# MDAnalysis/transport-analysis

Measured on AMD Instinct MI355X. Metric: VACF lag-points/sec (n_frames x n_atoms / s), higher is better.
Workload: dtype f64

## Files before the change

### transport_analysis_amd/csrc/wfft.hpp

```cpp
#pragma once
#include <hip/hip_runtime.h>

#include <type_traits>
#include <utility>

#include "fft_engine.hpp"

namespace ta {

#ifndef WF_NW_R0
#define WF_NW_R0 0
#define WF_NW_VAL 0
#endif

template <int LO, int HI, class F>
__device__ __forceinline__ void static_for_range(F&& f) {
    [&]<int... I>(std::integer_sequence<int, I...>) {
        (f(std::integral_constant<int, LO + I>{}), ...);
    }(std::make_integer_sequence<int, (HI > LO ? HI - LO : 0)>{});
}

typedef unsigned int wf_u32x4 __attribute__((ext_vector_type(4)));

#include "wfft_twist.inc"

template <>
struct Dft<3> {
    static __device__ __forceinline__ void run(cd (&v)[3]) {
        constexpr double kS3 = 0.86602540378443864676372317075294;
        const cd t = v[1] + v[2], d = v[1] - v[2];
        const cd m = cd{v[0].x - 0.5 * t.x, v[0].y - 0.5 * t.y};
        const cd e = cd{kS3 * d.y, -kS3 * d.x};
        v[0] = v[0] + t;
        v[1] = m + e;
        v[2] = m - e;
    }
};

template <int N>
struct DftOddTables;
template <>
struct DftOddTables<7> {
    static constexpr double c[3] = {0.62348980185873353053, -0.22252093395631440429, -0.90096886790241912624};
    static constexpr double s[3] = {0.78183148246802980871, 0.97492791218182360702, 0.43388373911755812048};
};
template <>
struct DftOddTables<9> {
    static constexpr double c[4] = {0.76604444311897803520, 0.17364817766693034885, -0.5, -0.93969262078590838405};
    static constexpr double s[4] = {0.64278760968653932632, 0.98480775301220805937, 0.86602540378443864676,
                                    0.34202014332566873304};
};
template <int N>
__device__ __forceinline__ void dft_odd(cd (&v)[N]) {
    constexpr int H = N / 2;
    using Tb = DftOddTables<N>;
    cd sp[H], dm[H];
#pragma unroll
    for (int j = 1; j <= H; ++j) {
        sp[j - 1] = v[j] + v[N - j];
        dm[j - 1] = v[j] - v[N - j];
    }
    const cd x0 = v[0];
    cd sum = x0;
#pragma unroll
    for (int j = 0; j < H; ++j) sum = sum + sp[j];
    v[0] = sum;
#pragma unroll
    for (int k = 1; k <= H; ++k) {
        double rx = x0.x, ry = x0.y, ix = 0.0, iy = 0.0;
#pragma unroll
        for (int j = 1; j <= H; ++j) {
            const int m = (j * k) % N;
            const double cm = m == 0 ? 1.0 : Tb::c[(m <= H ? m : N - m) - 1];
            const double sm = m == 0 ? 0.0 : m <= H ? Tb::s[m - 1] : -Tb::s[N - m - 1];
            rx = fma(cm, sp[j - 1].x, rx);
            ry = fma(cm, sp[j - 1].y, ry);
            ix = fma(sm, dm[j - 1].x, ix);
            iy = fma(sm, dm[j - 1].y, iy);
        }
        v[k] = cd{rx + iy, ry - ix};
        v[N - k] = cd{rx - iy, ry + ix};
    }
}
template <>
struct Dft<7> {
    static __device__ __forceinline__ void run(cd (&v)[7]) { dft_odd<7>(v); }
};
template <>
struct Dft<9> {
    static __device__ __forceinline__ void run(cd (&v)[9]) { dft_odd<9>(v); }
};

template <int N2>
__device__ __forceinline__ void dft_2x(cd (&v)[2 * N2]) {
    constexpr int N = 2 * N2;
    cd s[2][N2];
#pragma unroll
    for (int j2 = 0; j2 < N2; ++j2) {
        const cd a = v[(2 * j2) % N], b = v[(N2 + 2 * j2) % N];
        s[0][j2] = a + b;
        s[1][j2] = a - b;
    }
    Dft<N2>::run(s[0]);
    Dft<N2>::run(s[1]);
#pragma unroll
    for (int q = 0; q < N; ++q) v[q] = s[q % 2][q % N2];
}
template <>
struct Dft<14> {
    static __device__ __forceinline__ void run(cd (&v)[14]) { dft_2x<7>(v); }
};
template <>
struct Dft<18> {
    static __device__ __forceinline__ void run(cd (&v)[18]) { dft_2x<9>(v); }
};

template <>
struct Dft<6> {
    static __device__ __forceinline__ void run(cd (&v)[6]) {
        cd s[2][3];
#pragma unroll
        for (int j2 = 0; j2 < 3; ++j2) {
            const cd a = v[(2 * j2) % 6], b = v[(3 + 2 * j2) % 6];
            s[0][j2] = a + b;
            s[1][j2] = a - b;
        }
        Dft<3>::run(s[0]);
        Dft<3>::run(s[1]);
#pragma unroll
        for (int q = 0; q < 6; ++q) v[q] = s[q % 2][q % 3];
    }
};

template <>
struct Dft<12> {
    static __device__ __forceinline__ void run(cd (&v)[12]) {
        cd s[4][3];
#pragma unroll
        for (int j2 = 0; j2 < 3; ++j2) {
            cd t[4] = {v[(4 * j2) % 12], v[(3 + 4 * j2) % 12], v[(6 + 4 * j2) % 12], v[(9 + 4 * j2) % 12]};
            Dft<4>::run(t);
#pragma unroll
            for (int k1 = 0; k1 < 4; ++k1) s[k1][j2] = t[k1];
        }
#pragma unroll
        for (int k1 = 0; k1 < 4; ++k1) Dft<3>::run(s[k1]);
#pragma unroll
        for (int q = 0; q < 12; ++q) v[q] = s[q % 4][q % 3];
    }
};

template <>
struct Dft<10> {
    static __device__ __forceinline__ void run(cd (&v)[10]) {
        cd s[2][5];
#pragma unroll
        for (int j2 = 0; j2 < 5; ++j2) {
            const cd a = v[(2 * j2) % 10], b = v[(5 + 2 * j2) % 10];
            s[0][j2] = a + b;
            s[1][j2] = a - b;
        }
        Dft<5>::run(s[0]);
        Dft<5>::run(s[1]);
#pragma unroll
        for (int q = 0; q < 10; ++q) v[q] = s[q % 2][q % 5];
    }
};

template <>
struct Dft<20> {
    static __device__ __forceinline__ void run(cd (&v)[20]) {
        cd s[4][5];
#pragma unroll
        for (int j2 = 0; j2 < 5; ++j2) {
            cd t[4] = {v[(4 * j2) % 20], v[(5 + 4 * j2) % 20], v[(10 + 4 * j2) % 20], v[(15 + 4 * j2) % 20]};
            Dft<4>::run(t);
#pragma unroll
            for (int k1 = 0; k1 < 4; ++k1) s[k1][j2] = t[k1];
        }
#pragma unroll
        for (int k1 = 0; k1 < 4; ++k1) Dft<5>::run(s[k1]);
#pragma unroll
        for (int q = 0; q < 20; ++q) v[q] = s[q % 4][q % 5];
    }
};

constexpr int kWfStageRows = 14 + 8;
inline size_t wf_table_elems(int R0, int R) { return 2 * (size_t)R * R0 * 512 + kWfStageRows * 64; }
inline cd wf_tan_form(long num, long den) {
    const long double pi = 3.141592653589793238462643383279502884L;
    num %= den;
    if (4 * num == den) return cd{-0x1p200, 0x1p-200};
    if (4 * num == 3 * den) return cd{0x1p200, 0x1p-200};
    if (num == 0) return cd{0.0, 1.0};
    if (2 * num == den) return cd{0.0, -1.0};
    const long double h = 2.0L * pi * (long double)num / (long double)den;
    const long double c = cosl(h), sn = -sinl(h);
    return cd{(double)(sn / c), (double)c};
}
inline void wf_fill_table(int R0, int R, cd* a) {
    const long L = 2L * R * R0 * 512;
    const long double pi = 3.141592653589793238462643383279502884L;
    for (long n = 0; n < L; ++n) {
        if (n == 0) a[n] = cd{1.0, 0.0};
        else if (2 * n == L) a[n] = cd{-1.0, 0.0};
        else if (4 * n == L) a[n] = cd{0.0, -1.0};
        else if (4 * n == 3 * L) a[n] = cd{0.0, 1.0};
        else {
            const long double h = 2.0L * pi * (long double)n / (long double)L;
            a[n] = cd{(double)cosl(h), (double)-sinl(h)};
        }
    }
    for (int r = 1; r < 8; ++r)
        for (int l = 0; l < 64; ++l) {
            a[L + (r - 1) * 64 + l] = a[(L / 512) * l * r];
            a[L + (6 + r) * 64 + l] = a[(L / 64) * (l & 7) * r];
        }
    cd* t = a + L + 14 * 64;
    for (int l = 0; l < 64; ++l) {
        const long gb = 8 * (l >> 3), gc = 8 * (l & 7) + (l >> 3);
        const long g[2] = {gb, gc};
        for (int st = 0; st < 2; ++st) {
            t[(4 * st + 0) * 64 + l] = wf_tan_form(4 * g[st], 512);
            t[(4 * st + 1) * 64 + l] = wf_tan_form(2 * g[st], 512);
            t[(4 * st + 2) * 64 + l] = wf_tan_form(g[st], 512);
            t[(4 * st + 3) * 64 + l] = wf_tan_form(g[st] + 64, 512);
        }
    }
}

template <int R0_>
struct WPlan {
    static constexpr int R0 = R0_;
    static constexpr int N1 = 512;
    static constexpr int NW = R0 == WF_NW_R0 ? WF_NW_VAL : R0 <= 4 ? 2 : R0 <= 7 ? 4 : 8;
    static constexpr int NT = 64 * NW;
    static constexpr int K1 = (N1 + NT - 1) / NT;
#ifndef WF_SPREAD_ALL
    static constexpr bool kSpreadRows = R0 >= 9 && R0 <= 16;
#else
    static constexpr bool kSpreadRows = WF_SPREAD_ALL && (R0 < 18 || R0 == WF_NW_R0);
#endif
#ifndef WF_REG_EXCHANGE
    static constexpr bool kRegExchange = R0 >= 16;
#else
    static constexpr bool kRegExchange = WF_REG_EXCHANGE;
#endif
#ifndef WF_REG_EXCHANGE_SINGLE
    static constexpr bool kRegExchangeSingle = R0 == 2 || R0 == 7 || R0 == 9 || R0 == 10 || R0 == 12 || R0 == 14;
#else
    static constexpr bool kRegExchangeSingle = (WF_REG_EXCHANGE_SINGLE >> (R0 - 1)) & 1;
#endif
#ifndef WF_MINW_R0
    static __host__ __device__ constexpr int min_waves(bool , bool lng) { return R0 == 2 ? 4 : 1; }
#else
    static __host__ __device__ constexpr int min_waves(bool, bool) { return R0 == WF_MINW_R0 ? WF_MINW_VAL : 1; }
#endif
    static constexpr bool kTwResident = true;
    static constexpr int M = R0 * N1;
    static constexpr int NS1 = (R0 + NW - 1) / NW;
    static constexpr int NLO = R0 / NW, REM = R0 % NW;
    static __host__ __device__ constexpr int sub_count(int wave) { return NLO + (wave < REM ? 1 : 0); }
    static __host__ __device__ constexpr int sub_base(int wave) { return wave * NLO + (wave < REM ? wave : REM); }
    static constexpr size_t kLds = (size_t)M * sizeof(cd);

    struct RealSel {
        unsigned qmask[2];
        unsigned q1mask[2];
    };
    static __host__ __device__ constexpr int owner(int q) {
        for (int w = 0; w < NW; ++w)
            if (q >= sub_base(w) && q < sub_base(w) + sub_count(w)) return w;
        return 0;
    }
    static __host__ __device__ constexpr RealSel real_selection() {
        RealSel r{{0u, 0u}, {0u, 0u}};
        for (int t = 0; t < 2; ++t) {
            int load[8] = {0, 0, 0, 0, 0, 0, 0, 0}, simd[4] = {0, 0, 0, 0};
            auto take = [&](int q, bool self) {
                r.qmask[t] |= 1u << q;
                if (self) r.q1mask[t] |= 1u << q;
                ++load[owner(q)];
                ++simd[owner(q) % 4];
            };
            const int span = t == 0 ? R0 : R0 - 1;
            for (int q = 0; q < R0; ++q)
                if ((span - q + R0) % R0 == q) take(q, true);
            for (int q = 0; q < R0; ++q) {
                const int m = (span - q + R0) % R0;
                if (m <= q) continue;
                const int wa = owner(q), wb = owner(m);
                const int ca = 16 * load[wa] + simd[wa % 4], cb = 16 * load[wb] + simd[wb % 4];
                take(cb < ca ? m : q, false);
            }
        }
        return r;
    }
    static constexpr RealSel kRealSel = real_selection();
};

__device__ __forceinline__ cd wf_load(__amdgpu_buffer_rsrc_t r, unsigned lane_off, unsigned uni_off) {
    const wf_u32x4 v = __builtin_amdgcn_raw_buffer_load_b128(r, lane_off, uni_off, 0);
    return __builtin_bit_cast(cd, v);
}

struct WfSubPost {
    int lane, hi, lo;
    __device__ __forceinline__ explicit WfSubPost(int lane_) : lane(lane_) {
        asm volatile("" : "+v"(lane));
        hi = lane >> 3;
        lo = lane & 7;
    }
    __device__ __forceinline__ void read_a(const cd* __restrict__ reg, cd (&v)[8]) const {
#pragma unroll
        for (int n2 = 0; n2 < 8; ++n2) v[n2] = reg[64 * n2 + lane];
    }
    __device__ __forceinline__ void stage_a(cd* __restrict__ reg, cd (&v)[8], const cd (&twa)[7]) const {
        Dft<8>::run(v);
#pragma unroll
        for (int a = 1; a < 8; ++a) v[a] = cmul(v[a], twa[a - 1]);
        __builtin_amdgcn_wave_barrier();
#pragma unroll
        for (int a = 0; a < 8; ++a) reg[a * 64 + (lane ^ (8 * (a & 1)))] = v[a];
        __builtin_amdgcn_wave_barrier();
        const int base = hi * 64 + (lo ^ (8 * (hi & 1)));
#pragma unroll
        for (int n1 = 0; n1 < 8; ++n1) v[n1] = reg[base ^ (8 * n1)];
        __builtin_amdgcn_wave_barrier();
    }
    __device__ __forceinline__ void stage_b(cd* __restrict__ reg, cd (&v)[8], const cd (&twb)[7]) const {
        Dft<8>::run(v);
#pragma unroll
        for (int b = 1; b < 8; ++b) v[b] = cmul(v[b], twb[b - 1]);
        __builtin_amdgcn_wave_barrier();
        const int x = lo ^ hi;
#pragma unroll
        for (int b = 0; b < 8; ++b) reg[(hi * 8 + b) * 8 + (x ^ b)] = v[b];
        __builtin_amdgcn_wave_barrier();
#pragma unroll
        for (int n0 = 0; n0 < 8; ++n0) v[n0] = reg[lane * 8 + (n0 ^ x)];
        __builtin_amdgcn_wave_barrier();
    }
    __device__ __forceinline__ void stage_c(cd (&v)[8], double (&acc)[8]) const {
        Dft<8>::run(v);
#pragma unroll
        for (int c = 0; c < 8; ++c) acc[c] = fma(v[c].y, v[c].y, fma(v[c].x, v[c].x, acc[c]));
        __builtin_amdgcn_wave_barrier();
    }
};

template <int ROT>
__device__ __forceinline__ void wf_bf(cd& A, cd& B, const cd t) {
    const double qx = fma(-t.x, B.y, B.x), qy = fma(t.x, B.x, B.y);
    const cd a = A;
    if constexpr (ROT == 0) {
        A = cd{fma(t.y, qx, a.x), fma(t.y, qy, a.y)};
        B = cd{fma(-t.y, qx, a.x), fma(-t.y, qy, a.y)};
    } else {
        A = cd{fma(t.y, qy, a.x), fma(-t.y, qx, a.y)};
        B = cd{fma(-t.y, qy, a.x), fma(t.y, qx, a.y)};
    }
}
__device__ __forceinline__ void wf_dft8_tw(cd (&v)[8], const cd (&t)[4]) {
    wf_bf<0>(v[0], v[4], t[0]);
    wf_bf<0>(v[1], v[5], t[0]);
    wf_bf<0>(v[2], v[6], t[0]);
    wf_bf<0>(v[3], v[7], t[0]);
    wf_bf<0>(v[0], v[2], t[1]);
    wf_bf<0>(v[1], v[3], t[1]);
    wf_bf<1>(v[4], v[6], t[1]);
    wf_bf<1>(v[5], v[7], t[1]);
    wf_bf<0>(v[0], v[1], t[2]);
    wf_bf<1>(v[2], v[3], t[2]);
    wf_bf<0>(v[4], v[5], t[3]);
    wf_bf<1>(v[6], v[7], t[3]);
    const cd y4 = v[1], y6 = v[3], y1 = v[4], y3 = v[6];
    v[1] = y1, v[3] = y3, v[4] = y4, v[6] = y6;
}

struct WfTw {
    cd b[4], c[4];
};
typedef unsigned wf_u32pair __attribute__((ext_vector_type(2)));
__device__ __forceinline__ void wf_transpose_hi(cd (&v)[8]) {
    unsigned w[8][4];
#pragma unroll
    for (int a = 0; a < 8; ++a) {
        const wf_u32x4 t = __builtin_bit_cast(wf_u32x4, v[a]);
        w[a][0] = t.x, w[a][1] = t.y, w[a][2] = t.z, w[a][3] = t.w;
    }
#pragma unroll
    for (int a = 0; a < 8; ++a)
        if (!(a & 4))
#pragma unroll
            for (int d = 0; d < 4; ++d) {
                const wf_u32pair r = __builtin_amdgcn_permlane32_swap(w[a][d], w[a | 4][d], false, false);
                w[a][d] = r.x, w[a | 4][d] = r.y;
            }
#pragma unroll
    for (int a = 0; a < 8; ++a)
        if (!(a & 2))
#pragma unroll
            for (int d = 0; d < 4; ++d) {
                const wf_u32pair r = __builtin_amdgcn_permlane16_swap(w[a][d], w[a | 2][d], false, false);
                w[a][d] = r.x, w[a | 2][d] = r.y;
            }
#pragma unroll
    for (int a = 0; a < 8; ++a)
        if (!(a & 1))
#pragma unroll
            for (int d = 0; d < 4; ++d) {
                const unsigned lo = w[a][d], hi = w[a | 1][d];
                w[a][d] = __builtin_amdgcn_update_dpp(lo, hi, 0x128, 0xF, 0xC, false);
                w[a | 1][d] = __builtin_amdgcn_update_dpp(hi, lo, 0x128, 0xF, 0x3, false);
            }
#pragma unroll
    for (int a = 0; a < 8; ++a) {
        wf_u32x4 t;
        t.x = w[a][0], t.y = w[a][1], t.z = w[a][2], t.w = w[a][3];
        v[a] = __builtin_bit_cast(cd, t);
    }
}

struct WfAddr {
    unsigned we, wo, re, ro, x16, b2w, b2r;
    __device__ __forceinline__ void init(int lane, unsigned q_bytes) {
        const int hi = lane >> 3, lo = lane & 7;
        we = q_bytes + 16u * (unsigned)lane;
        wo = q_bytes + 16u * (unsigned)(lane ^ 8);
        const unsigned rb = q_bytes + 16u * (unsigned)(hi * 64 + lo);
        re = rb + 128u * (unsigned)(hi & 1);
        ro = rb - 128u * (unsigned)(hi & 1);
        x16 = 16u * (unsigned)(hi ^ lo);
        b2w = q_bytes + 1024u * (unsigned)hi;
        b2r = b2w + 128u * (unsigned)lo;
    }
    __device__ __forceinline__ unsigned w2(int k) const { return (x16 ^ (16u * (unsigned)k)) + b2w; }
    __device__ __forceinline__ unsigned r2(int k) const { return (x16 ^ (16u * (unsigned)k)) + b2r; }
};
struct WfSub {
    const WfAddr& ad;
    unsigned char* smem;
    __device__ __forceinline__ WfSub(const WfAddr& ad_, unsigned char* smem_) : ad(ad_), smem(smem_) {}
    __device__ __forceinline__ cd& at(unsigned base, unsigned off) const {
        return *reinterpret_cast<cd*>(__builtin_assume_aligned(smem + (base + off), 16));
    }
    template <unsigned SO>
    __device__ __forceinline__ void read_a(cd (&v)[8]) const {
#pragma unroll
        for (int n2 = 0; n2 < 8; ++n2) v[n2] = at(ad.we, SO + 1024u * n2);
    }
    template <unsigned SO>
    __device__ __forceinline__ void stage_a_w(cd (&v)[8]) const {
        Dft<8>::run(v);
        __builtin_amdgcn_wave_barrier();
#pragma unroll
        for (int a = 0; a < 8; ++a) at(a & 1 ? ad.wo : ad.we, SO + 1024u * a) = v[a];
        __builtin_amdgcn_wave_barrier();
    }
    template <unsigned SO>
    __device__ __forceinline__ void stage_a_r(cd (&v)[8]) const {
        __builtin_amdgcn_wave_barrier();
#pragma unroll
        for (int n1 = 0; n1 < 8; ++n1) v[n1] = at(n1 & 1 ? ad.ro : ad.re, SO + 128u * n1);
        __builtin_amdgcn_wave_barrier();
    }
    template <unsigned SO, bool XV = false>
    __device__ __forceinline__ void stage_a(cd (&v)[8]) const {
        if constexpr (XV) {
            Dft<8>::run(v);
            wf_transpose_hi(v);
        } else {
            stage_a_w<SO>(v);
            stage_a_r<SO>(v);
        }
    }
    template <unsigned SO>
    __device__ __forceinline__ void stage_b_w(cd (&v)[8], const WfTw& tw) const {
        wf_dft8_tw(v, tw.b);
        __builtin_amdgcn_wave_barrier();
#pragma unroll
        for (int b = 0; b < 8; ++b) at(ad.w2(b), SO + 128u * b) = v[b];
        __builtin_amdgcn_wave_barrier();
    }
    template <unsigned SO>
    __device__ __forceinline__ void stage_b_r(cd (&v)[8]) const {
        __builtin_amdgcn_wave_barrier();
#pragma unroll
        for (int n0 = 0; n0 < 8; ++n0) v[n0] = at(ad.r2(n0), SO);
        __builtin_amdgcn_wave_barrier();
    }
    template <unsigned SO>
    __device__ __forceinline__ void stage_b(cd (&v)[8], const WfTw& tw) const {
        stage_b_w<SO>(v, tw);
        stage_b_r<SO>(v);
    }
    __device__ __forceinline__ void stage_c(cd (&v)[8], const WfTw& tw, double (&acc)[8]) const {
        wf_dft8_tw(v, tw.c);
#pragma unroll
        for (int c = 0; c < 8; ++c) acc[c] = fma(v[c].y, v[c].y, fma(v[c].x, v[c].x, acc[c]));
    }
    __device__ __forceinline__ void stage_c_w(cd (&v)[8], const WfTw& tw, double (&acc)[8], double wgt) const {
        wf_dft8_tw(v, tw.c);
#pragma unroll
        for (int c = 0; c < 8; ++c) acc[c] = fma(wgt, fma(v[c].y, v[c].y, v[c].x * v[c].x), acc[c]);
    }
};

constexpr unsigned kWfSubBytes = 512 * sizeof(cd);

struct WfNoHook {
    template <class T>
    __device__ __forceinline__ void operator()(T) const {}
};
template <int I>
using wf_part = std::integral_constant<int, I>;

template <int S0, bool XV = false, class Hook = WfNoHook>
__device__ __forceinline__ void wf_sub512(const WfSub& w, const WfTw& tw, double (&acc)[8], Hook&& hook = Hook{}) {
    cd v[8];
    w.read_a<S0 * kWfSubBytes>(v);
    hook(wf_part<0>{});
    w.template stage_a<S0 * kWfSubBytes, XV>(v);
    hook(wf_part<1>{});
    w.stage_b<S0 * kWfSubBytes>(v, tw);
    hook(wf_part<2>{});
    w.stage_c(v, tw, acc);
    hook(wf_part<3>{});
}

template <int S0, bool XV = false>
__device__ __forceinline__ void wf_sub512_w(const WfSub& w, const WfTw& tw, double (&acc)[8], double wgt) {
    cd v[8];
    w.read_a<S0 * kWfSubBytes>(v);
    w.template stage_a<S0 * kWfSubBytes, XV>(v);
    w.stage_b<S0 * kWfSubBytes>(v, tw);
    w.stage_c_w(v, tw, acc, wgt);
}

template <int S0, bool XV = false, class Hook = WfNoHook>
__device__ __forceinline__ void wf_sub512_x2(const WfSub& w, const WfTw& tw, double (&acc0)[8],
                                             double (&acc1)[8], Hook&& hook = Hook{}) {
    constexpr unsigned A = S0 * kWfSubBytes, B = A + kWfSubBytes;
    cd v0[8], v1[8];
    w.read_a<A>(v0);
    w.read_a<B>(v1);
    __builtin_amdgcn_wave_barrier();
    hook(wf_part<0>{});
    w.template stage_a<A>(v0);
    w.template stage_a<B, XV>(v1);
    hook(wf_part<1>{});
    w.stage_b<A>(v0, tw);
    w.stage_b<B>(v1, tw);
    hook(wf_part<2>{});
    w.stage_c(v0, tw, acc0);
    w.stage_c(v1, tw, acc1);
    hook(wf_part<3>{});
}

template <bool XV = false, class Hook = WfNoHook>
__device__ __forceinline__ void wf_sub512_x3(const WfSub& w, const WfTw& tw, double (&acc0)[8],
                                             double (&acc1)[8], double (&acc2)[8], Hook&& hook = Hook{}) {
    constexpr unsigned A = 0, B = kWfSubBytes, C = 2 * kWfSubBytes;
    cd v0[8], v1[8], v2[8];
    w.read_a<A>(v0);
    w.read_a<B>(v1);
    w.read_a<C>(v2);
    __builtin_amdgcn_wave_barrier();
    hook(wf_part<0>{});
    w.template stage_a<A>(v0);
    w.template stage_a<B>(v1);
    w.template stage_a<C, XV>(v2);
    hook(wf_part<1>{});
    w.stage_b<A>(v0, tw);
    w.stage_b<B>(v1, tw);
    w.stage_b<C>(v2, tw);
    hook(wf_part<2>{});
    w.stage_c(v0, tw, acc0);
    w.stage_c(v1, tw, acc1);
    w.stage_c(v2, tw, acc2);
    hook(wf_part<3>{});
}

__device__ __forceinline__ void wf_unit_of(long atom, int k, int D, long* pair, int* kind) {
    const long c0 = atom * D;
    if (D == 2) {
        *pair = atom, *kind = 2;
    } else if (D == 1) {
        *pair = c0 >> 1, *kind = (int)(c0 & 1);
    } else if ((c0 & 1) == 0) {
        *pair = (c0 >> 1) + k, *kind = k == 0 ? 2 : 0;
    } else {
        *pair = (c0 >> 1) + k, *kind = k == 0 ? 1 : 2;
    }
}

typedef unsigned int wf_u32x2 __attribute__((__vector_size__(2 * sizeof(unsigned int))));

__device__ __forceinline__ cd wf_cfma(cd acc, cd a, cd b) {
    return {acc.x + (a.x * b.x - a.y * b.y), acc.y + (a.x * b.y + a.y * b.x)};
}

template <bool S, class A, class B>
__device__ __forceinline__ auto& wf_pick(A& a, B& b) {
    if constexpr (S) return a;
    else return b;
}

template <class P, bool BYP = false, bool LONG = false, bool STAMP = false, bool SRC32 = false>
__global__ void __launch_bounds__(P::NT, P::min_waves(BYP, LONG))
    k_wsplit_accum(const double* __restrict__ pm, long pitch, int T, long n_units,
                   const cd* __restrict__ tw2, double* __restrict__ accg, int D, int R_arg,
                   unsigned long long* __restrict__ stamps) {
    extern __shared__ __attribute__((aligned(16))) unsigned char smem_raw[];
    cd* lds = reinterpret_cast<cd*>(smem_raw);
    constexpr int R0 = P::R0, N1 = P::N1, NW = P::NW, NS1 = P::NS1, M = P::M;
    static_assert(!(SRC32 && LONG), "float32 slabs: plans without an outer radix only");
    const int R = LONG ? R_arg : 1, npass = 2 * R, L = npass * M;
    const int tid = threadIdx.x, wave = tid >> 6;
    int lane = tid & 63;
    const int bi = blockIdx.x >> 3;
    const int pass = bi % npass;
    const long tuple = (blockIdx.x & 7) + 8 * (bi / npass), n_tuples = gridDim.x / npass;
    const int upa = BYP ? (D == 3 ? 2 : 1) : 1;
    const int grp = BYP && (D & 1) ? 2 : 1;

    double acc[NS1][8];
#pragma unroll
    for (int s = 0; s < NS1; ++s)
#pragma unroll
        for (int c = 0; c < 8; ++c) acc[s][c] = 0.0;
    unsigned long long st_acc[4] = {0, 0, 0, 0}, st_prev = 0, st_t0 = 0, st_r0 = 0, st_tail = 0, st_s2end = 0;
    if constexpr (STAMP) {
        st_prev = st_t0 = __builtin_amdgcn_s_memtime();
        st_r0 = __builtin_amdgcn_s_memrealtime();
    }
#define WF_STAMP(i)                                                   \
    if constexpr (STAMP) {                                            \
        const unsigned long long now_ = __builtin_amdgcn_s_memtime(); \
        st_acc[i] += now_ - st_prev;                                  \
        st_prev = now_;                                               \
    }
    const __amdgpu_buffer_rsrc_t twr =
        __builtin_amdgcn_make_buffer_rsrc(const_cast<cd*>(tw2), 0, (L + kWfStageRows * 64) * 16, 0x00020000);
    auto unit_rsrc = [&](long item, int k, int* kind) {
        long pair = item;
        const bool live = item < n_units;
        *kind = 2;
        if constexpr (BYP) wf_unit_of(live ? item : 0, k, D, &pair, kind);
        if constexpr (SRC32)
            return __builtin_amdgcn_make_buffer_rsrc(
                const_cast<float*>(reinterpret_cast<const float*>(pm) + (live ? pair : 0) * pitch * 2), 0,
                live ? T * 8 : 0, 0x00020000);
        else
            return __builtin_amdgcn_make_buffer_rsrc(const_cast<double*>(pm + (live ? pair : 0) * pitch * 2), 0,
                                                     live ? T * 16 : 0, 0x00020000);
    };
    using RowT = std::conditional_t<SRC32, wf_u32x2, cd>;
    auto load_row = [&](__amdgpu_buffer_rsrc_t rs, int kd, int u, unsigned row_off) -> RowT {
        if constexpr (SRC32) {
            return __builtin_amdgcn_raw_buffer_load_b64(rs, (unsigned)u * 8u, row_off * 8u, 0);
        } else {
            if (!BYP || kd == 2) return wf_load(rs, (unsigned)u * 16u, row_off * 16u);
            return cd{__builtin_bit_cast(double, __builtin_amdgcn_raw_buffer_load_b64(
                                                     rs, (unsigned)u * 16u + (unsigned)kd * 8u, row_off * 16u, 0)),
                      0.0};
        }
    };
    [[maybe_unused]] auto wf_widen = [&](wf_u32x2 r, int kd) {
        if (!BYP || kd == 2)
            return cd{(double)__builtin_bit_cast(float, (unsigned)r[0]), (double)__builtin_bit_cast(float, (unsigned)r[1])};
        return cd{(double)__builtin_bit_cast(float, (unsigned)(kd ? r[1] : r[0])), 0.0};
    };
    constexpr int K1 = P::K1, NT = P::NT;
    RowT xx[K1][R0];
    auto issue_loads = [&](__amdgpu_buffer_rsrc_t rs, int kd) {
#pragma unroll
        for (int k1 = 0; k1 < K1; ++k1) {
            const int u = tid + NT * k1;
            if (K1 * NT != N1 && u >= N1) continue;
            if (!BYP || kd == 2) {
#pragma unroll
                for (int j = 0; j < R0; ++j) xx[k1][j] = load_row(rs, 2, u, (unsigned)(N1 * j));
            } else {
#pragma unroll
                for (int j = 0; j < R0; ++j) xx[k1][j] = load_row(rs, kd, u, (unsigned)(N1 * j));
            }
        }
    };
#ifndef WF_LOAD_PARTS
#define WF_LOAD_PARTS 4
#endif
    constexpr int NR = K1 * R0;
    constexpr bool kSpread = P::kSpreadRows || (SRC32 && R0 >= 18);
#ifndef WF_SPREAD32_TAIL
#define WF_SPREAD32_TAIL 0
#endif
    constexpr int NSPREAD = WF_LOAD_PARTS != 4 ? 0 : (kSpread ? (SRC32 && R0 >= 18 ? NR - WF_SPREAD32_TAIL : NR) : 0);
    auto issue_row = [&](auto ii, __amdgpu_buffer_rsrc_t rs, int kd) {
        constexpr int i = decltype(ii)::value, k1 = i / R0, j = i % R0;
        const int u = tid + NT * k1;
        if (K1 * NT != N1 && u >= N1) return;
        if (!BYP || kd == 2) xx[k1][j] = load_row(rs, 2, u, (unsigned)(N1 * j));
        else xx[k1][j] = load_row(rs, kd, u, (unsigned)(N1 * j));
    };
    auto issue_loads_part = [&](auto part_c, __amdgpu_buffer_rsrc_t rs, int kd) {
        constexpr int PART = decltype(part_c)::value;
        static_for_range<PART * NSPREAD / 4, (PART + 1) * NSPREAD / 4>([&](auto ii) { issue_row(ii, rs, kd); });
    };
    auto issue_loads_tail = [&](__amdgpu_buffer_rsrc_t rs, int kd) {
        static_for_range<NSPREAD, NR>([&](auto ii) { issue_row(ii, rs, kd); });
    };
    int kind = 2, nkind = 2;
    __amdgpu_buffer_rsrc_t crs = unit_rsrc(tuple * grp, 0, &kind);
    issue_loads(crs, kind);
    WfTw stw;
    auto load_stage_tw = [&]() {
#pragma unroll
        for (int a = 0; a < 4; ++a) {
            stw.b[a] = wf_load(twr, (unsigned)lane * 16u, (unsigned)(L + (14 + a) * 64) * 16u);
            stw.c[a] = wf_load(twr, (unsigned)lane * 16u, (unsigned)(L + (18 + a) * 64) * 16u);
        }
    };
    constexpr bool kTwRes = P::kTwResident && !(BYP && LONG && R0 >= 18);
    if constexpr (kTwRes) load_stage_tw();
    WfAddr wad;
    wad.init(lane, (unsigned)P::sub_base(wave) * kWfSubBytes);
    const WfSub wsub(wad, smem_raw);
    int k = 0;
    bool zero_pending = false;
    for (long item = tuple * grp; item < n_units;) {
#ifndef WF_REAL_S1_SKIP
#define WF_REAL_S1_SKIP 0
#endif
        const unsigned qsel = (WF_REAL_S1_SKIP && BYP && kind != 2) ? P::kRealSel.qmask[pass ? 1 : 0] : ~0u;
#pragma unroll
        for (int k1 = 0; k1 < K1; ++k1) {
        const int u = tid + NT * k1;
        if (K1 * NT != N1 && u >= N1) continue;
        [[maybe_unused]] cd xwide[SRC32 ? R0 : 1];
        if constexpr (SRC32) {
#pragma unroll
            for (int j = 0; j < R0; ++j) xwide[j] = wf_widen(xx[k1][j], kind);
        }
        cd(&x)[R0] = wf_pick<SRC32>(xwide, xx[k1]);
        cd g, g2, h;
        auto load_seeds = [&]() {
            g = wf_load(twr, (unsigned)(u * R) * 32u, 0u);
            g2 = wf_load(twr, (unsigned)(u * R) * 64u, 0u);
            h = wf_load(twr, (unsigned)(u * pass) * 16u, 0u);
        };
        if constexpr (!LONG) load_seeds();
        if constexpr (LONG) {
            const int sj = pass * N1, so = pass * M;
            if (pass) {
                int idx = 0;
#pragma unroll
                for (int j = 1; j < R0; ++j) {
                    idx += sj;
                    idx -= idx >= L ? L : 0;
                    x[j] = cmul(x[j], tw_uniform(tw2, idx));
                }
            }
            auto outer_rows = [&](auto single) {
                int base = 0;
                for (int jo = 1; jo < R; ++jo) {
                    base += so;
                    base -= base >= L ? L : 0;
                    if (jo * M >= T) break;
                    int idx = base;
                    constexpr int NZ = 10;
#pragma unroll
                    for (int j0 = 0; j0 < R0; j0 += NZ) {
                        cd z[NZ];
#pragma unroll
                        for (int i = 0; i < NZ; ++i)
                            if (j0 + i < R0)
                                z[i] = load_row(crs, decltype(single)::value ? kind : 2, u, (unsigned)(N1 * (j0 + i) + M * jo));
#pragma unroll
                        for (int i = 0; i < NZ; ++i)
                            if (j0 + i < R0) {
                                x[j0 + i] = wf_cfma(x[j0 + i], z[i], tw_uniform(tw2, idx));
                                idx += sj;
                                idx -= idx >= L ? L : 0;
                            }
                        __builtin_amdgcn_sched_barrier(0);
                    }
                }
            };
            if (BYP && kind != 2) outer_rows(std::true_type{});
            else outer_rows(std::false_type{});
            __builtin_amdgcn_sched_barrier(0);
            load_seeds();
        } else if (pass) {
#pragma unroll
            for (int j = 1; j < R0; ++j) x[j] = cmul(x[j], cd{WfTwist<R0>::re(j), WfTwist<R0>::im(j)});
        }
        Dft<R0>::run(x);
        {
            cd te = pass ? h : cd{1.0, 0.0};
            cd to = pass ? cmul(h, g) : g;
            if (pass) x[0] = cmul(x[0], te);
            if (!(WF_REAL_S1_SKIP && BYP) || (qsel & 1u)) lds[u] = x[0];
            if constexpr (R0 > 1) {
                x[1] = cmul(x[1], to);
                if (!(WF_REAL_S1_SKIP && BYP) || (qsel & 2u)) lds[N1 + u] = x[1];
            }
#pragma unroll
            for (int q = 2; q < R0; ++q) {
                if (q & 1) {
                    to = cmul(to, g2);
                    x[q] = cmul(x[q], to);
                } else {
                    te = cmul(te, g2);
                    x[q] = cmul(x[q], te);
                }
                if (!(WF_REAL_S1_SKIP && BYP) || (qsel >> q & 1u)) lds[q * N1 + u] = x[q];
            }
        }
        }
        if constexpr (!kTwRes) {
            asm volatile("" : "+v"(lane));
            load_stage_tw();
        }
        WF_STAMP(0)
        __syncthreads();
        if (BYP && zero_pending) {
#pragma unroll
            for (int s = 0; s < NS1; ++s)
#pragma unroll
                for (int c = 0; c < 8; ++c) acc[s][c] = 0.0;
            zero_pending = false;
        }
        const bool last_of_item = !BYP || k == upa - 1;
        long nitem = item;
        if (last_of_item) {
            if (BYP && grp == 2 && (item & 1) == 0 && item + 1 < n_units) nitem = item + 1;
            else nitem = (item & ~(long)(grp - 1)) + grp * n_tuples;
        }
        const int nk = last_of_item ? 0 : k + 1;
        const __amdgpu_buffer_rsrc_t nrs = unit_rsrc(nitem, nk, &nkind);
        auto row_hook = [&](auto part_c) {
#if WF_LOAD_PARTS == 4
            issue_loads_part(part_c, nrs, nkind);
#endif
        };
        if (BYP && kind != 2) {
            const int wv = __builtin_amdgcn_readfirstlane(wave);
            static_for_range<0, 4>([&](auto part_c) { row_hook(part_c); });
            const unsigned qs = P::kRealSel.qmask[pass ? 1 : 0] >> P::sub_base(wv);
            const unsigned q1 = P::kRealSel.q1mask[pass ? 1 : 0] >> P::sub_base(wv);
            static_for_range<0, NS1>([&](auto ss) {
                constexpr int s = decltype(ss)::value;
                if ((s < P::NLO || wv < P::REM) && (qs >> s & 1u))
                    wf_sub512_w<s, P::kRegExchangeSingle>(wsub, stw, acc[s], (q1 >> s & 1u) ? 1.0 : 2.0);
            });
        } else
        if constexpr (NS1 == 3 && P::NLO == 2 && P::REM != 0) {
            if constexpr (SRC32) {
                if (wave < P::REM) wf_sub512_x3<P::kRegExchange>(wsub, stw, acc[0], acc[1], acc[2], row_hook);
                else wf_sub512_x2<0, P::kRegExchange>(wsub, stw, acc[0], acc[1], row_hook);
            } else {
                if (wave < P::REM) wf_sub512_x3<P::kRegExchange>(wsub, stw, acc[0], acc[1], acc[2]);
                else wf_sub512_x2<0, P::kRegExchange>(wsub, stw, acc[0], acc[1]);
            }
        } else {
            static_for_range<0, NS1>([&](auto ss) {
                constexpr int s = decltype(ss)::value;
                constexpr bool full = s < P::NLO;
                constexpr bool nfull = s + 1 < P::NLO;
                constexpr bool head = full && nfull && (s % 2 == 0);
                constexpr bool tail = full && s > 0 && (s % 2 == 1);
                if constexpr (head) {
                    if constexpr (s == 0) wf_sub512_x2<s, P::kRegExchange>(wsub, stw, acc[s], acc[s + 1], row_hook);
                    else wf_sub512_x2<s, P::kRegExchange>(wsub, stw, acc[s], acc[s + 1]);
                } else if constexpr (!tail) {
                    if constexpr (s == 0) wf_sub512<s, P::kRegExchangeSingle>(wsub, stw, acc[s], row_hook);
                    else if (full || wave < P::REM) wf_sub512<s, P::kRegExchangeSingle>(wsub, stw, acc[s]);
                }
            });
        }
        if constexpr (STAMP) st_s2end = __builtin_amdgcn_s_memtime();
        const int wv = __builtin_amdgcn_readfirstlane(wave);
        auto store_acc = [&](long row) {
            const __amdgpu_buffer_rsrc_t sr = __builtin_amdgcn_make_buffer_rsrc(
                accg + (row * npass + pass) * (long)M, 0, M * 8, 0x00020000);
#pragma unroll
            for (int s = 0; s < NS1; ++s) {
                const int q = P::sub_base(wv) + s;
                if (s < P::NLO || wv < P::REM) {
#pragma unroll
                    for (int c2 = 0; c2 < 4; ++c2) {
                        const cd two{acc[s][2 * c2], acc[s][2 * c2 + 1]};
                        __builtin_amdgcn_raw_buffer_store_b128(__builtin_bit_cast(wf_u32x4, two), sr, (unsigned)lane * 16u,
                                                               (unsigned)((q * 4 + c2) * 64) * 16u, 0);
                    }
                }
            }
        };
        if constexpr (BYP) {
            if (last_of_item) {
                store_acc(item);
                zero_pending = true;
            }
        } else {
            if (nitem >= n_units) store_acc(tuple);
        }
        __builtin_amdgcn_sched_barrier(0);
        issue_loads_tail(nrs, nkind);
        kind = nkind, item = nitem, k = nk, crs = nrs;
        if constexpr (STAMP) st_tail += __builtin_amdgcn_s_memtime() - st_s2end;
        WF_STAMP(1)
        __syncthreads();
    }
    if constexpr (!BYP) {
        if (tuple * grp >= n_units) {
            const int wv = __builtin_amdgcn_readfirstlane(wave);
            const __amdgpu_buffer_rsrc_t sr = __builtin_amdgcn_make_buffer_rsrc(
                accg + (tuple * npass + pass) * (long)M, 0, M * 8, 0x00020000);
#pragma unroll
            for (int s = 0; s < NS1; ++s) {
                const int q = P::sub_base(wv) + s;
                if (s < P::sub_count(wv)) {
#pragma unroll
                    for (int c2 = 0; c2 < 4; ++c2)
                        __builtin_amdgcn_raw_buffer_store_b128(__builtin_bit_cast(wf_u32x4, cd{0.0, 0.0}), sr,
                                                               (unsigned)lane * 16u, (unsigned)((q * 4 + c2) * 64) * 16u, 0);
                }
            }
        }
    }
    if constexpr (STAMP) {
        st_acc[2] = __builtin_amdgcn_s_memtime() - st_t0;
        st_acc[3] = __builtin_amdgcn_s_memrealtime() - st_r0;
        if (lane == 0 && (wave == 0 || wave == NW / 2)) {
            for (int i = 0; i < 4; ++i) stamps[16 * (long)blockIdx.x + (wave ? 4 : 0) + i] = st_acc[i];
            stamps[16 * (long)blockIdx.x + 8 + (wave ? 1 : 0)] = st_tail;
        }
    }
#undef WF_STAMP
}

struct WfSubT {
    int lane, hi, lo;
    __device__ __forceinline__ explicit WfSubT(int lane_) : lane(lane_) {
        asm volatile("" : "+v"(lane));
        hi = lane >> 3;
        lo = lane & 7;
    }
    __device__ __forceinline__ void run(cd* __restrict__ reg, cd (&v)[8], const cd (&twa)[7],
                                        const cd (&twb)[7]) const {
        Dft<8>::run(v);
#pragma unroll
        for (int n0 = 1; n0 < 8; ++n0) v[n0] = cmul(v[n0], twb[n0 - 1]);
        __builtin_amdgcn_wave_barrier();
        const int x = lo ^ hi;
#pragma unroll
        for (int n0 = 0; n0 < 8; ++n0) reg[(hi * 8 + n0) * 8 + (x ^ n0)] = v[n0];
        __builtin_amdgcn_wave_barrier();
#pragma unroll
        for (int b = 0; b < 8; ++b) v[b] = reg[lane * 8 + (b ^ x)];
        __builtin_amdgcn_wave_barrier();
        Dft<8>::run(v);
        __builtin_amdgcn_wave_barrier();
        const int base = hi * 64 + (lo ^ (8 * (hi & 1)));
#pragma unroll
        for (int n1 = 0; n1 < 8; ++n1) reg[base ^ (8 * n1)] = v[n1];
        __builtin_amdgcn_wave_barrier();
#pragma unroll
        for (int a = 0; a < 8; ++a) v[a] = reg[a * 64 + (lane ^ (8 * (a & 1)))];
        __builtin_amdgcn_wave_barrier();
#pragma unroll
        for (int a = 1; a < 8; ++a) v[a] = cmul(v[a], twa[a - 1]);
        Dft<8>::run(v);
        __builtin_amdgcn_wave_barrier();
#pragma unroll
        for (int n2 = 0; n2 < 8; ++n2) reg[64 * n2 + lane] = v[n2];
        __builtin_amdgcn_wave_barrier();
    }
};



template <class P, bool LONG = false, int PF = 0>
__global__ void __launch_bounds__(P::NT)
    k_winverse(const double* __restrict__ spec, int T, long n_items, const cd* __restrict__ tw2,
               double* __restrict__ out, long ld, int R_arg) {
    extern __shared__ __attribute__((aligned(16))) unsigned char smem_raw[];
    cd* lds = reinterpret_cast<cd*>(smem_raw);
    constexpr int R0 = P::R0, N1 = P::N1, NW = P::NW, NT = P::NT, K1 = P::K1, M = P::M, NSA = P::NS1;
    static_assert(!LONG || PF == 0, "the spectrum prefetch is for the single-transform case");
    static_assert(PF <= NSA, "prefetch depth counts sub-series of a wave");
    const int R = LONG ? R_arg : 1, L = 2 * R * M;
    int tid = threadIdx.x, lane = tid & 63;
    const int wave = tid >> 6;
    const __amdgpu_buffer_rsrc_t twr =
        __builtin_amdgcn_make_buffer_rsrc(const_cast<cd*>(tw2), 0, (L + kWfStageRows * 64) * 16, 0x00020000);
    cd v[NSA][8];
    auto load_spec = [&](long item, int cp, int s) {
        const int wv = __builtin_amdgcn_readfirstlane(wave);
        const int q = wv + NW * s;
        const bool live = item < n_items && q < R0;
        const __amdgpu_buffer_rsrc_t sr = __builtin_amdgcn_make_buffer_rsrc(
            const_cast<double*>(spec + (live ? item : 0) * (long)L + (long)(2 * cp) * M), 0, live ? 2 * M * 8 : 0,
            0x00020000);
#pragma unroll
        for (int c2 = 0; c2 < 4; ++c2) {
            const cd a = wf_load(sr, (unsigned)lane * 16u, (unsigned)((q * 4 + c2) * 64) * 16u);
            const cd b = wf_load(sr, (unsigned)lane * 16u, (unsigned)(M / 2 + (q * 4 + c2) * 64) * 16u);
            v[s][2 * c2] = cd{a.x, b.x};
            v[s][2 * c2 + 1] = cd{a.y, b.y};
        }
    };
    constexpr bool kHoistNorm = !LONG && R0 >= 9;
    double rnorm[kHoistNorm ? K1 : 1][kHoistNorm ? R0 : 1];
    if constexpr (kHoistNorm) {
#pragma unroll
        for (int k1 = 0; k1 < K1; ++k1)
#pragma unroll
            for (int j = 0; j < R0; ++j) {
                const int n = tid + NT * k1 + N1 * j;
                rnorm[k1][j] = n < T ? 1.0 / (2.0 * (double)M * (double)(T - n)) : 0.0;
            }
    }
#pragma unroll
    for (int s = 0; s < PF; ++s) load_spec(blockIdx.x, 0, s);
    for (long item = blockIdx.x; item < n_items; item += gridDim.x) {
        for (int cp = 0; cp < R; ++cp) {
            asm volatile("" : "+v"(tid), "+v"(lane));
            {
                cd twa[7], twb[7];
#pragma unroll
                for (int a = 0; a < 7; ++a) {
                    twa[a] = wf_load(twr, (unsigned)lane * 16u, (unsigned)(L + a * 64) * 16u);
                    twb[a] = wf_load(twr, (unsigned)lane * 16u, (unsigned)(L + (7 + a) * 64) * 16u);
                }
#pragma unroll
                for (int s = PF; s < NSA; ++s) load_spec(item, cp, s);
                const WfSubT wt(lane);
#pragma unroll
                for (int s = 0; s < NSA; ++s) {
                    const int q = wave + NW * s;
                    if (NW * s + NW - 1 < R0 || q < R0) wt.run(lds + q * N1, v[s], twa, twb);
                }
            }
            __syncthreads();
            if constexpr (PF > 0) {
                __builtin_amdgcn_sched_barrier(0);
#pragma unroll
                for (int s = 0; s < PF; ++s) load_spec(item + gridDim.x, 0, s);
                __builtin_amdgcn_sched_barrier(0);
            }
            cd xx[K1][R0];
#pragma unroll
            for (int k1 = 0; k1 < K1; ++k1) {
                const int u = tid + NT * k1;
                if (K1 * NT != N1 && u >= N1) continue;
                cd(&x)[R0] = xx[k1];
                const cd g = wf_load(twr, (unsigned)(u * R) * 32u, 0u), g2 = wf_load(twr, (unsigned)(u * R) * 64u, 0u);
#pragma unroll
                for (int q = 0; q < R0; ++q) x[q] = lds[q * N1 + u];
                cd te = cd{1.0, 0.0}, to = g;
                if constexpr (R0 > 1) x[1] = cmul(x[1], to);
#pragma unroll
                for (int q = 2; q < R0; ++q) {
                    if (q & 1) {
                        to = cmul(to, g2);
                        x[q] = cmul(x[q], to);
                    } else {
                        te = cmul(te, g2);
                        x[q] = cmul(x[q], te);
                    }
                }
                Dft<R0>::run(x);
            }
            __builtin_amdgcn_wave_barrier();
#pragma unroll
            for (int k1 = 0; k1 < K1; ++k1) {
                const int u = tid + NT * k1;
                if (K1 * NT != N1 && u >= N1) continue;
#pragma unroll
                for (int j = 0; j < R0; ++j) lds[u + N1 * j] = xx[k1][j];
            }
            __syncthreads();
            double* o = out + item * ld;
#pragma unroll
            for (int k1 = 0; k1 < K1; ++k1) {
                const int u = tid + NT * k1;
                if (K1 * NT != N1 && u >= N1) continue;
                cd(&x)[R0] = xx[k1];
                const int mu = u == 0 ? 0 : N1 - u;
                if constexpr (!LONG) {
                    const cd h = wf_load(twr, (unsigned)u * 16u, 0u);
#pragma unroll
                    for (int j = 0; j < R0; ++j) {
                        const int n = u + N1 * j;
                        const int jm = u == 0 ? (R0 - j) % R0 : R0 - 1 - j;
                        const cd qm = lds[mu + N1 * jm];
                        const cd w = j == 0 ? h : cmul(h, cd{WfTwist<R0>::re(j), WfTwist<R0>::im(j)});
                        const double ar = 0.5 * (x[j].x + qm.x), br = 0.5 * (x[j].y + qm.y),
                                     bi = -0.5 * (x[j].x - qm.x);
                        const double lagv = ar + (w.x * br - w.y * bi);
                        if constexpr (kHoistNorm) {
                            if (n < T) o[n] = lagv * rnorm[k1][j];
                        } else {
                            if (n < T) o[n] = lagv / (2.0 * (double)M * (double)(T - n));
                        }
                    }
                } else {
                    const int c0 = 2 * cp, c1 = c0 + 1;
                    const cd h0 = wf_load(twr, (unsigned)(u * c0) * 16u, 0u),
                             h1 = wf_load(twr, (unsigned)(u * c1) * 16u, 0u);
                    const bool first = cp == 0, last = cp == R - 1;
                    int j0 = 0, j1 = 0;
#pragma unroll
                    for (int j = 0; j < R0; ++j) {
                        const int jm = u == 0 ? (R0 - j) % R0 : R0 - 1 - j;
                        const cd qm = lds[mu + N1 * jm];
                        const cd qa = cd{0.5 * (x[j].x + qm.x), 0.5 * (x[j].y - qm.y)};
                        const cd qb = cd{0.5 * (x[j].y + qm.y), -0.5 * (x[j].x - qm.x)};
                        int i0 = j0, i1 = j1;
                        for (int jo = 0; jo < R; ++jo) {
                            const int n = u + N1 * j + M * jo;
                            const cd w0 = cmul(h0, tw_uniform(tw2, i0)), w1 = cmul(h1, tw_uniform(tw2, i1));
                            double a = (w0.x * qa.x - w0.y * qa.y) + (w1.x * qb.x - w1.y * qb.y);
                            if (n < T) {
                                if (!first) a += o[n];
                                o[n] = last ? a / ((double)L * (double)(T - n)) : a;
                            }
                            i0 += c0 * M, i0 -= i0 >= L ? L : 0;
                            i1 += c1 * M, i1 -= i1 >= L ? L : 0;
                        }
                        j0 += c0 * N1, j0 -= j0 >= L ? L : 0;
                        j1 += c1 * N1, j1 -= j1 >= L ? L : 0;
                    }
                }
            }
            __syncthreads();
        }
    }
}

struct W1 {
    static constexpr int NT = 256, NWV = 4, M = 512;
    static constexpr size_t kLds = (size_t)NWV * 2 * 512 * sizeof(cd);
};

template <bool SINGLE>
__device__ __forceinline__ void w1_two_passes(cd* __restrict__ regA, cd* __restrict__ regB, int lane,
                                              const cd (&twa)[7], const cd (&twb)[7], const cd (&v)[8],
                                              const cd (&tB)[8], double (&accA)[8], double (&accB)[8]) {
    const WfSubPost w(lane);
    if constexpr (SINGLE) {
        cd a[8];
#pragma unroll
        for (int n2 = 0; n2 < 8; ++n2) a[n2] = v[n2];
        w.stage_a(regA, a, twa);
        w.stage_b(regA, a, twb);
        w.stage_c(a, accA);
        return;
    }
    cd a[8], b[8];
#pragma unroll
    for (int n2 = 0; n2 < 8; ++n2) {
        a[n2] = v[n2];
        b[n2] = cmul(v[n2], tB[n2]);
    }
    w.stage_a(regA, a, twa);
    w.stage_a(regB, b, twa);
    w.stage_b(regA, a, twb);
    w.stage_b(regB, b, twb);
    w.stage_c(a, accA);
    w.stage_c(b, accB);
}

template <bool SINGLE, int PACK>
__global__ void __launch_bounds__(W1::NT)
    k_w1_accum(const double* __restrict__ pm, long pitch, int T, long n_pairs,
               const cd* __restrict__ tw2, double* __restrict__ accg) {
    static_assert(PACK == 1 || (SINGLE && (PACK == 2 || PACK == 4 || PACK == 8)), "packing needs the one-pass form");
    extern __shared__ __attribute__((aligned(16))) unsigned char smem_raw[];
    cd* lds = reinterpret_cast<cd*>(smem_raw);
    const int tid = threadIdx.x, lane = tid & 63, wave = tid >> 6;
    const long gw = (long)blockIdx.x * W1::NWV + wave, nw = (long)gridDim.x * W1::NWV;
    cd* regA = lds + wave * 1024;
    cd* regB = regA + 512;
    const __amdgpu_buffer_rsrc_t twr = __builtin_amdgcn_make_buffer_rsrc(
        const_cast<cd*>(tw2), 0, (2 * W1::M + kWfStageRows * 64) * 16, 0x00020000);
    cd twa[7], twb[7], tB[8];
#pragma unroll
    for (int a = 0; a < 7; ++a) {
        twa[a] = wf_load(twr, (unsigned)lane * 16u, (unsigned)(2 * W1::M + a * 64) * 16u);
        twb[a] = wf_load(twr, (unsigned)lane * 16u, (unsigned)(2 * W1::M + (7 + a) * 64) * 16u);
    }
#pragma unroll
    for (int n2 = 0; n2 < 8; ++n2) tB[n2] = wf_load(twr, (unsigned)lane * 16u, (unsigned)(64 * n2) * 16u);
    double accA[8], accB[8];
#pragma unroll
    for (int c = 0; c < 8; ++c) accA[c] = accB[c] = 0.0;
    constexpr int kPer = 8 / PACK;
    for (long p = gw; p * PACK < n_pairs; p += nw) {
        cd v[8];
#pragma unroll
        for (int q = 0; q < PACK; ++q) {
            const long pair = p * PACK + q;
            const __amdgpu_buffer_rsrc_t rs = __builtin_amdgcn_make_buffer_rsrc(
                const_cast<double*>(pm + (pair < n_pairs ? pair : 0) * pitch * 2), 0, pair < n_pairs ? T * 16 : 0, 0x00020000);
#pragma unroll
            for (int j = 0; j < kPer; ++j) v[q * kPer + j] = wf_load(rs, (unsigned)lane * 16u, (unsigned)(64 * j) * 16u);
        }
        w1_two_passes<SINGLE>(regA, regB, lane, twa, twb, v, tB, accA, accB);
    }
    double* out = accg + gw * 2 * W1::M;
#pragma unroll
    for (int c = 0; c < 8; ++c) {
        const int sb = (lane >> 3) + 8 * (lane & 7) + 64 * c;
        out[2 * sb] = SINGLE ? 2.0 * accA[c] : accA[c];
        out[2 * sb + 1] = SINGLE ? 0.0 : accB[c];
    }
}

template <bool SINGLE>
__global__ void __launch_bounds__(W1::NT)
    k_w1_bp(const double* __restrict__ pm, long pitch, int T, long n_atoms, int D,
            const cd* __restrict__ tw2, double* __restrict__ out, long ld) {
    extern __shared__ __attribute__((aligned(16))) unsigned char smem_raw[];
    cd* lds = reinterpret_cast<cd*>(smem_raw);
    const int tid = threadIdx.x, lane = tid & 63, wave = tid >> 6;
    const long gw = (long)blockIdx.x * W1::NWV + wave, nw = (long)gridDim.x * W1::NWV;
    cd* regA = lds + wave * 1024;
    cd* regB = regA + 512;
    const __amdgpu_buffer_rsrc_t twr = __builtin_amdgcn_make_buffer_rsrc(
        const_cast<cd*>(tw2), 0, (2 * W1::M + kWfStageRows * 64) * 16, 0x00020000);
    cd twa[7], twb[7], tB[8];
#pragma unroll
    for (int a = 0; a < 7; ++a) {
        twa[a] = wf_load(twr, (unsigned)lane * 16u, (unsigned)(2 * W1::M + a * 64) * 16u);
        twb[a] = wf_load(twr, (unsigned)lane * 16u, (unsigned)(2 * W1::M + (7 + a) * 64) * 16u);
    }
#pragma unroll
    for (int n2 = 0; n2 < 8; ++n2) tB[n2] = wf_load(twr, (unsigned)lane * 16u, (unsigned)(64 * n2) * 16u);
    const int n_units = D == 3 ? 2 : 1;
    auto forward = [&](long atom, double (&accA)[8], double (&accB)[8]) __attribute__((always_inline)) {
        auto unit_of = [&](int k, long* pair, int* kind) {
            const long c0 = atom * D;
// ... 112 lines not shown
```

Measured before the change: 110.3 billion.

## Specialize FFT accumulation kernel per pass with folded twist and derived seeds

Splits the accumulation kernel body into compile-time pass variants (pass 0 and pass 1) for the non-bypass, non-long plans with radix 18 or 20, selecting the variant by block index. Pass 1 folds the half-sample input twist into specialised twisted DFT-18/20 butterflies, which removes the per-element twiddle multiplies. Seed twiddles g and g2 are now computed by complex squaring instead of being loaded from the table, and pass 0 skips the multiplies by one. The cost is two inlined copies of the body, which enlarges the code and may change register allocation, and squaring the seeds could introduce small rounding differences.

```diff
diff --git a/transport_analysis_amd/csrc/wfft.hpp b/transport_analysis_amd/csrc/wfft.hpp
--- a/transport_analysis_amd/csrc/wfft.hpp
+++ b/transport_analysis_amd/csrc/wfft.hpp
@@ -182,6 +182,57 @@
         for (int k1 = 0; k1 < 4; ++k1) Dft<5>::run(s[k1]);
 #pragma unroll
         for (int q = 0; q < 20; ++q) v[q] = s[q % 4][q % 5];
+    }
+};
+
+template <int R0>
+struct DftTwisted {
+    static constexpr bool kHave = false;
+};
+template <int R0>
+__device__ __forceinline__ cd wf_twist_in(const cd (&v)[R0], int n, int n2) {
+    const cd x = v[n % R0];
+    return ((n >= R0 ? 1 : 0) + n2) & 1 ? cd{-x.x, -x.y} : x;
+}
+template <>
+struct DftTwisted<18> {
+    static constexpr bool kHave = true;
+    static __device__ __forceinline__ void run(cd (&v)[18]) {
+        cd s[2][9];
+#pragma unroll
+        for (int j2 = 0; j2 < 9; ++j2) {
+            const cd a = wf_twist_in<18>(v, 2 * j2, j2), b = wf_twist_in<18>(v, 9 + 2 * j2, j2);
+            s[0][j2] = cd{a.x + b.y, a.y - b.x};
+            s[1][j2] = cd{a.x - b.y, a.y + b.x};
+        }
+        Dft<9>::run(s[0]);
+        Dft<9>::run(s[1]);
+#pragma unroll
+        for (int q = 0; q < 18; ++q) v[q] = s[q % 2][(q % 9 + 5) % 9];
+    }
+};
+template <>
+struct DftTwisted<20> {
+    static constexpr bool kHave = true;
+    static __device__ __forceinline__ void run(cd (&v)[20]) {
+        cd s[4][5];
+#pragma unroll
+        for (int j2 = 0; j2 < 5; ++j2) {
+            const cd a = wf_twist_in<20>(v, 4 * j2, j2), b = wf_twist_in<20>(v, 5 + 4 * j2, j2);
+            const cd c = wf_twist_in<20>(v, 10 + 4 * j2, j2), d = wf_twist_in<20>(v, 15 + 4 * j2, j2);
+            const cd p = cd{a.x + c.y, a.y - c.x}, m = cd{a.x - c.y, a.y + c.x};
+            const cd e = cd{b.x + d.y, b.y - d.x}, f = cd{b.x - d.y, b.y + d.x};
+            const double ex = e.x + e.y, ey = e.y - e.x;
+            const double fx = f.y - f.x, fy = f.x + f.y;
+            s[0][j2] = cd{fma(kR2, ex, p.x), fma(kR2, ey, p.y)};
+            s[2][j2] = cd{fma(-kR2, ex, p.x), fma(-kR2, ey, p.y)};
+            s[1][j2] = cd{fma(kR2, fx, m.x), fma(-kR2, fy, m.y)};
+            s[3][j2] = cd{fma(-kR2, fx, m.x), fma(kR2, fy, m.y)};
+        }
+#pragma unroll
+        for (int k1 = 0; k1 < 4; ++k1) Dft<5>::run(s[k1]);
+#pragma unroll
+        for (int q = 0; q < 20; ++q) v[q] = s[q % 4][(q % 5 + 3) % 5];
     }
 };
 
@@ -607,20 +658,34 @@
     else return b;
 }
 
-template <class P, bool BYP = false, bool LONG = false, bool STAMP = false, bool SRC32 = false>
-__global__ void __launch_bounds__(P::NT, P::min_waves(BYP, LONG))
-    k_wsplit_accum(const double* __restrict__ pm, long pitch, int T, long n_units,
-                   const cd* __restrict__ tw2, double* __restrict__ accg, int D, int R_arg,
-                   unsigned long long* __restrict__ stamps) {
-    extern __shared__ __attribute__((aligned(16))) unsigned char smem_raw[];
+#ifndef WF_PASS_SPLIT
+#define WF_PASS_SPLIT 1
+#endif
+#ifndef WF_SEED_DERIVE
+#define WF_SEED_DERIVE 2
+#endif
+#ifndef WF_TWIST_FOLD
+#define WF_TWIST_FOLD 1
+#endif
+template <class P, bool BYP, bool LONG, bool SRC32>
+constexpr bool wf_pass_split = WF_PASS_SPLIT && !BYP && !LONG && !SRC32 && (P::R0 == 18 || P::R0 == 20);
+
+__device__ __forceinline__ cd wf_csqr(cd a) { return {a.x * a.x - a.y * a.y, 2.0 * (a.x * a.y)}; }
+
+template <class P, bool BYP, bool LONG, bool STAMP, bool SRC32, int PASS>
+__device__ __forceinline__ void wf_accum_body(unsigned char* smem_raw, const double* __restrict__ pm, long pitch, int T,
+                                              long n_units, const cd* __restrict__ tw2, double* __restrict__ accg, int D,
+                                              int R_arg, unsigned long long* __restrict__ stamps) {
     cd* lds = reinterpret_cast<cd*>(smem_raw);
     constexpr int R0 = P::R0, N1 = P::N1, NW = P::NW, NS1 = P::NS1, M = P::M;
     static_assert(!(SRC32 && LONG), "float32 slabs: plans without an outer radix only");
+    static_assert(PASS < 0 || (!BYP && !LONG), "a compile-time pass: lag sums without an outer radix");
     const int R = LONG ? R_arg : 1, npass = 2 * R, L = npass * M;
     const int tid = threadIdx.x, wave = tid >> 6;
     int lane = tid & 63;
     const int bi = blockIdx.x >> 3;
-    const int pass = bi % npass;
+    const int pass = PASS >= 0 ? PASS : bi % npass;
+    constexpr bool kTwistFold = PASS == 1 && WF_TWIST_FOLD && DftTwisted<R0>::kHave;
     const long tuple = (blockIdx.x & 7) + 8 * (bi / npass), n_tuples = gridDim.x / npass;
     const int upa = BYP ? (D == 3 ? 2 : 1) : 1;
     const int grp = BYP && (D & 1) ? 2 : 1;
@@ -746,9 +811,15 @@
         cd(&x)[R0] = wf_pick<SRC32>(xwide, xx[k1]);
         cd g, g2, h;
         auto load_seeds = [&]() {
-            g = wf_load(twr, (unsigned)(u * R) * 32u, 0u);
-            g2 = wf_load(twr, (unsigned)(u * R) * 64u, 0u);
-            h = wf_load(twr, (unsigned)(u * pass) * 16u, 0u);
+            if constexpr (PASS == 1 && WF_SEED_DERIVE >= 1) {
+                h = wf_load(twr, (unsigned)u * 16u, 0u);
+                g = wf_csqr(h);
+            } else {
+                g = wf_load(twr, (unsigned)(u * R) * 32u, 0u);
+                if (PASS != 0) h = wf_load(twr, (unsigned)(u * pass) * 16u, 0u);
+            }
+            if constexpr ((PASS == 0 && WF_SEED_DERIVE >= 2) || (PASS == 1 && WF_SEED_DERIVE >= 3)) g2 = wf_csqr(g);
+            else g2 = wf_load(twr, (unsigned)(u * R) * 64u, 0u);
         };
         if constexpr (!LONG) load_seeds();
         if constexpr (LONG) {
@@ -793,14 +864,23 @@
             __builtin_amdgcn_sched_barrier(0);
             load_seeds();
         } else if (pass) {
-#pragma unroll
-            for (int j = 1; j < R0; ++j) x[j] = cmul(x[j], cd{WfTwist<R0>::re(j), WfTwist<R0>::im(j)});
-        }
-        Dft<R0>::run(x);
+            if constexpr (!kTwistFold) {
+#pragma unroll
+                for (int j = 1; j < R0; ++j) x[j] = cmul(x[j], cd{WfTwist<R0>::re(j), WfTwist<R0>::im(j)});
+            }
+        }
+        if constexpr (kTwistFold) DftTwisted<R0>::run(x);
+        else Dft<R0>::run(x);
         {
-            cd te = pass ? h : cd{1.0, 0.0};
-            cd to = pass ? cmul(h, g) : g;
-            if (pass) x[0] = cmul(x[0], te);
+            cd te, to;
+            if constexpr (PASS == 0) {
+                te = cd{1.0, 0.0};
+                to = g;
+            } else {
+                te = pass ? h : cd{1.0, 0.0};
+                to = pass ? cmul(h, g) : g;
+                if (pass) x[0] = cmul(x[0], te);
+            }
             if (!(WF_REAL_S1_SKIP && BYP) || (qsel & 1u)) lds[u] = x[0];
             if constexpr (R0 > 1) {
                 x[1] = cmul(x[1], to);
@@ -812,7 +892,7 @@
                     to = cmul(to, g2);
                     x[q] = cmul(x[q], to);
                 } else {
-                    te = cmul(te, g2);
+                    te = (PASS == 0 && q == 2) ? g2 : cmul(te, g2);
                     x[q] = cmul(x[q], te);
                 }
                 if (!(WF_REAL_S1_SKIP && BYP) || (qsel >> q & 1u)) lds[q * N1 + u] = x[q];
@@ -941,6 +1021,26 @@
 #undef WF_STAMP
 }
 
+template <class P, bool BYP = false, bool LONG = false, bool STAMP = false, bool SRC32 = false>
+__global__ void __launch_bounds__(P::NT, P::min_waves(BYP, LONG))
+    k_wsplit_accum(const double* __restrict__ pm, long pitch, int T, long n_units,
+                   const cd* __restrict__ tw2, double* __restrict__ accg, int D, int R_arg,
+                   unsigned long long* __restrict__ stamps) {
+    extern __shared__ __attribute__((aligned(16))) unsigned char smem_raw[];
+    if constexpr (wf_pass_split<P, BYP, LONG, SRC32>) {
+#ifdef WF_FIX_PASS
+        wf_accum_body<P, BYP, LONG, STAMP, SRC32, WF_FIX_PASS>(smem_raw, pm, pitch, T, n_units, tw2, accg, D, R_arg, stamps);
+        return;
+#endif
+        if ((blockIdx.x >> 3) & 1)
+            wf_accum_body<P, BYP, LONG, STAMP, SRC32, 1>(smem_raw, pm, pitch, T, n_units, tw2, accg, D, R_arg, stamps);
+        else
+            wf_accum_body<P, BYP, LONG, STAMP, SRC32, 0>(smem_raw, pm, pitch, T, n_units, tw2, accg, D, R_arg, stamps);
+    } else {
+        wf_accum_body<P, BYP, LONG, STAMP, SRC32, -1>(smem_raw, pm, pitch, T, n_units, tw2, accg, D, R_arg, stamps);
+    }
+}
+
 struct WfSubT {
     int lane, hi, lo;
     __device__ __forceinline__ explicit WfSubT(int lane_) : lane(lane_) {
```

Result: faster. 115.5 billion, median of 6 (+4.7%).
